# Justin-Huber/SfM-project

Measured on AMD Instinct MI355X. Metric: verified matches/sec (match+RANSAC), higher is better.
Workload: dtype int8 MFMA -> exact int32 (K1), f32 (K2); 1 GPU; cfg4: all 124750 unordered pairs of 500 synthetic images x 4096 128-D u8 SIFT-like descriptors; L2 match (mutual cross check + ratio 4/5) + 8-point RANSAC 4096 hyp/pair (seed 42, Sampson 1 px^2, min 15 inliers); launches of <= 131072 pairs; n_img=500, k=4096, n_hyp=4096, pairs_total=124750, pairs_rank0=124750, launches_rank0=1, parallelism=pair-sharded dp1

## Files before the change

include/sfmcore.h:

```cpp
#ifndef SFMCORE_H
#define SFMCORE_H

#include <stdint.h>

#ifdef __cplusplus
extern "C" {
#endif

#define SFM_OK 0
#define SFM_ERR_INVALID (-1)
#define SFM_ERR_HIP (-2)
#define SFM_ERR_NOMEM (-3)

#define SFM_METRIC_L2 0
#define SFM_METRIC_HAMMING 1

#define SFM_XC_NONE 0
#define SFM_XC_MUTUAL 1
#define SFM_XC_OPENCV 2

typedef struct sfm_ctx sfm_ctx;

typedef struct sfm_match_params {
    int32_t metric;
// ... 118 lines not shown
               int32_t* out_n_tracks, int32_t* out_track_ptr, int32_t* out_track_img,
               int32_t* out_track_kp);

int sfm_triangulate(sfm_ctx* ctx, int32_t n_cam, const double* cams, const double* pp,
                    int32_t n_pt, const int32_t* pt_ptr, const int32_t* cam_idx, const double* uv,
                    double* out_pts, double* out_stats);

typedef struct sfm_register_params {
    int32_t n_hyp;
    int32_t refine;
    double thr;
    uint64_t seed;
} sfm_register_params;

int sfm_register_batch(sfm_ctx* ctx, int32_t n_img, const int32_t* corr_ptr, const double* xy,
                       const double* X, const double* intr, const int32_t* img_id,
                       const sfm_register_params* prm, double* out_cams, int32_t* out_count,
                       int32_t* out_key, uint8_t* out_mask);

typedef struct sfm_orb_params {
    int32_t n_features;
    int32_t n_levels;
    double scale_factor;
    int32_t fast_threshold;
    int32_t _pad;
} sfm_orb_params;

int sfm_orb_batch(sfm_ctx* ctx, const uint8_t* images, int32_t n_img, int32_t H, int32_t W,
                  const sfm_orb_params* prm, float* out_kp, uint8_t* out_desc,
                  int32_t* out_count);

int sfm_calib_mfma_i8(sfm_ctx* ctx, float target_ms, double* out);

#ifdef __cplusplus
}
#endif
#endif
```

sfm-project_amd/csrc/capi.hip:

```cpp
#include "sfm_internal.h"

static thread_local std::string g_err;

namespace sfm {
void set_error(const std::string& msg) { g_err = msg; }

void* workspace(sfm_ctx* ctx, size_t bytes) {
    ctx->rs_last_w = nullptr;
    ctx->rs_last_pairs = ctx->rs_last_hyp = 0;
    if (bytes <= ctx->ws_bytes) return ctx->ws;
    hipStreamCaptureStatus cap = hipStreamCaptureStatusNone;
    if (hipStreamIsCapturing(ctx->stream, &cap) == hipSuccess && cap != hipStreamCaptureStatusNone) {
        set_error("workspace growth to " + std::to_string(bytes) +
                  " bytes while the context's stream is being captured: run the call once "
                  "uncaptured first so the workspace is sized");
        return nullptr;
    }
    if (ctx->ws) {
        (void)hipStreamSynchronize(ctx->stream);
        (void)hipFree(ctx->ws);
        ctx->ws = nullptr;
        ctx->ws_bytes = 0;
    }
    size_t want = align_up(bytes + bytes / 4, 1 << 20);
// ... 24 lines not shown
    if (std::string(prop.gcnArchName).rfind("gfx950", 0) != 0) {
        sfm::set_error(std::string("sfm_ctx_create: libsfmcore is built for gfx950, device is ") +
                       prop.gcnArchName);
        return SFM_ERR_INVALID;
    }
    sfm_ctx* c = new sfm_ctx();
    c->device = device;
    c->n_cu = prop.multiProcessorCount;
    if (hipStreamCreateWithFlags(&c->own_stream, hipStreamNonBlocking) != hipSuccess) {
        delete c;
        sfm::set_error("sfm_ctx_create: hipStreamCreate failed");
        return SFM_ERR_HIP;
    }
    if (hipEventCreateWithFlags(&c->handoff, hipEventDisableTiming) != hipSuccess) {
        (void)hipStreamDestroy(c->own_stream);
        delete c;
        sfm::set_error("sfm_ctx_create: hipEventCreate failed");
        return SFM_ERR_HIP;
    }
    c->stream = c->own_stream;
    *out = c;
    return SFM_OK;
}

int sfm_ctx_destroy(sfm_ctx* ctx) {
    if (!ctx) return SFM_OK;
    (void)hipSetDevice(ctx->device);
    if (ctx->stream) (void)hipStreamSynchronize(ctx->stream);
    if (ctx->ws) (void)hipFree(ctx->ws);
    if (ctx->handoff) (void)hipEventDestroy(ctx->handoff);
    if (ctx->pinned) (void)hipHostFree(ctx->pinned);
    if (ctx->poll_ev) (void)hipEventDestroy(ctx->poll_ev);
    if (ctx->rs_acc) (void)hipFree(ctx->rs_acc);
    if (ctx->own_stream) (void)hipStreamDestroy(ctx->own_stream);
    delete ctx;
    return SFM_OK;
}

int sfm_ctx_set_stream(sfm_ctx* ctx, void* hip_stream) {
    SFM_REQUIRE(ctx != nullptr, "sfm_ctx_set_stream: ctx is NULL");
    hipStream_t s = (hipStream_t)hip_stream;
    if (s == ctx->stream) return SFM_OK;
    SFM_HIP_CHECK(hipSetDevice(ctx->device));
    SFM_HIP_CHECK(hipEventRecord(ctx->handoff, ctx->stream));
    SFM_HIP_CHECK(hipStreamWaitEvent(s, ctx->handoff, 0));
    ctx->stream = s;
    return SFM_OK;
}

int sfm_ctx_sync(sfm_ctx* ctx) {
    SFM_REQUIRE(ctx != nullptr, "sfm_ctx_sync: ctx is NULL");
    SFM_HIP_CHECK(hipSetDevice(ctx->device));
    SFM_HIP_CHECK(hipStreamSynchronize(ctx->stream));
    return SFM_OK;
}

int sfm_match_batch(sfm_ctx* ctx, const uint8_t* desc, const int32_t* n_kp, int32_t n_img,
                    int32_t k_max, int32_t dim, const int32_t* pairs, int32_t n_pairs,
                    const sfm_match_params* prm, int32_t* out_count, int32_t* out_match,
                    int32_t* out_dist) {
    SFM_REQUIRE(ctx && prm, "sfm_match_batch: ctx/prm is NULL");
    SFM_REQUIRE(n_pairs >= 0 && n_img >= 0 && k_max >= 0, "sfm_match_batch: negative size");
    if (n_pairs == 0) return SFM_OK;
    SFM_REQUIRE(desc && n_kp && pairs && out_count && out_match && out_dist,
                "sfm_match_batch: NULL array");
    SFM_REQUIRE(prm->cross_check >= 0 && prm->cross_check <= 2, "sfm_match_batch: bad cross_check");
// ... 54 lines not shown
```

sfm-project_amd/csrc/match_l2fr.hip:

```cpp
#include <algorithm>
#include <climits>
#include <cstdlib>

#include "match_common.h"

namespace {

typedef int v4i __attribute__((ext_vector_type(4)));
typedef int v16i __attribute__((ext_vector_type(16)));
typedef __attribute__((address_space(3))) void lds_void;
typedef const __attribute__((address_space(1))) void gbl_void;

constexpr int D = 128;
#ifndef L2FR_WAVES
#define L2FR_WAVES 8
#endif
constexpr int WAVES = L2FR_WAVES;
constexpr int SCAN_THREADS = 64 * WAVES;
#ifndef L2FR_QT
#define L2FR_QT 4
#endif
constexpr int QT = L2FR_QT;
constexpr int QB = WAVES * QT * 32;
constexpr int SCAN_MIN_WAVES = 8 / QT;
// ... 677 lines not shown
            crec[tid] = fw[q];
            cA[tid] = norm[(size_t)a * k_pad + q];
        }
        __syncthreads();
        for (int c = g; c < nbat; c += 8) {
            const int q = cq[c];
            const int4 r = crec[c];
            const int row = (r.z - tg) * 32 + t, j = r.z * 32 + t;
            const uint4* x = &qrows[c * SLOTS];
            const uint4* y = &tiles[row * SLOTS];
            int dot = 0;
#pragma unroll
            for (int k = 0; k < SLOTS; ++k) {
                const uint4 u = x[k], v = y[k ^ (row & 7)];
                dot = __builtin_amdgcn_sdot4((int)u.x, (int)v.x, dot, false);
                dot = __builtin_amdgcn_sdot4((int)u.y, (int)v.y, dot, false);
                dot = __builtin_amdgcn_sdot4((int)u.z, (int)v.z, dot, false);
                dot = __builtin_amdgcn_sdot4((int)u.w, (int)v.w, dot, false);
            }
            const bool hit = (j < nb) && (dot + tci[row] == r.x);
            const unsigned long long bal = __ballot(hit);
            const unsigned m = (unsigned)(bal >> (32 * (g & 1)));
            if (t == 0 && m == 0) qs[q] = make_int4(ST_SLOW, 0, 0, 0);
            if (m != 0 && t == __builtin_ctz(m)) {
                const long long A = cA[c];
                const long long d1 = A - (2LL * dot - tnb[row]);
                const long long d2lo = r.y > E_VALID ? A - 2LL * r.y - 1 : sfm::DIST_INF;
                const long long d2hi = r.y > E_VALID ? A - 2LL * r.y : sfm::DIST_INF;
                int st;
                if (max_dist >= 0 && !(d1 < max_dist)) st = ST_DROP;
                else if (sfm::ratio_ok(d1, d2lo, rnum, rden, true)) st = ST_PASS;
                else if (!sfm::ratio_ok(d1, d2hi, rnum, rden, true)) st = ST_DROP;
                else st = ST_SLOW;
                qs[q] = make_int4(st, j, (int)d1, 0);
            }
        }
        __syncthreads();
    }
}

#ifndef L2FR_REC_SB
#define L2FR_REC_SB 2
#endif
constexpr int REC_SB = L2FR_REC_SB;
__global__ __launch_bounds__(256, REC_SB > 2 ? 2 : 3) void l2fr_recover_mfma_kernel(
    const uint8_t* __restrict__ desc, int k_max, int k_pad, const int32_t* __restrict__ norm,
    const int32_t* __restrict__ cinit, const int4* __restrict__ rinfo,
    const int32_t* __restrict__ n_rng, const int4* __restrict__ fwd,
    const uint8_t* __restrict__ cls, int rnum, int rden, long long max_dist,
    int4* __restrict__ qst) {
    __shared__ unsigned short clist[REC_R * KMAX];
    __shared__ __attribute__((aligned(16))) int gini[GROUP];
    __shared__ unsigned char gpar[GROUP];
    __shared__ unsigned long long wlo[4], whi[4];
    __shared__ int toff[9];
    const int ri = blockIdx.x, grp = blockIdx.y, tid = threadIdx.x;
    if (ri >= *n_rng) return;
    const int wave = tid >> 6, lane = tid & 63, h = lane >> 5, r32 = lane & 31;
    int4 pi[REC_R];
#pragma unroll
    for (int e = 0; e < REC_R; ++e) pi[e] = rinfo[(size_t)ri * REC_R + e];
    const int b = pi[0].z, nb = pi[0].w >> 16;
    const int ntiles = (nb + 31) >> 5, tg = grp * 8;
    if (nb <= 0 || tg >= ntiles) return;
    const uint8_t* db = desc + (size_t)b * k_max * D;

    uint4 cv[REC_R];
// ... 126 lines not shown
#pragma unroll
            for (int u = 0; u < 2; ++u) {
                v16i acc;
                const int* gi = gini + (2 * wave + u) * 32 + 4 * h;
#pragma unroll
                for (int g = 0; g < 4; ++g) {
                    const v4i c4 = *(const v4i*)(gi + 8 * g);
                    acc[4 * g + 0] = c4.x; acc[4 * g + 1] = c4.y;
                    acc[4 * g + 2] = c4.z; acc[4 * g + 3] = c4.w;
                }
#pragma unroll
                for (int s = 0; s < NK; ++s)
                    acc = __builtin_amdgcn_mfma_i32_32x32x32_i8(af[u][s], bf[k][s], acc, 0, 0, 0);
#pragma unroll
                for (int rr = 0; rr < 16; ++rr)
                    hit = (mine == u && acc[rr] == r.x) ? 8 * (rr >> 2) + 4 * h + (rr & 3) : hit;
            }
            hit = max(hit, __shfl_xor(hit, 32));
            if (h == 0 && qq[k] >= 0) {
                int4* qs = qst + (size_t)pp[k] * k_pad;
                if (hit < 0) {
                    qs[qq[k]] = make_int4(ST_SLOW, 0, 0, 0);
                } else {
                    const int jg = (2 * wave + mine) * 32 + hit;
                    const long long A = AA[k];
                    const long long d1 = A - 2LL * r.x - gpar[jg];
                    const long long d2lo = r.y > E_VALID ? A - 2LL * r.y - 1 : sfm::DIST_INF;
                    const long long d2hi = r.y > E_VALID ? A - 2LL * r.y : sfm::DIST_INF;
                    int st;
                    if (max_dist >= 0 && !(d1 < max_dist)) st = ST_DROP;
                    else if (sfm::ratio_ok(d1, d2lo, rnum, rden, true)) st = ST_PASS;
                    else if (!sfm::ratio_ok(d1, d2hi, rnum, rden, true)) st = ST_DROP;
                    else st = ST_SLOW;
                    qs[qq[k]] = make_int4(st, tg * 32 + jg, (int)d1, 0);
                }
            }
        }
    }
}

__global__ __launch_bounds__(256) void l2fr_compact_kernel(
    const uint8_t* __restrict__ desc, const int32_t* __restrict__ n_kp, int k_max, int k_pad,
    const int32_t* __restrict__ norm, const int32_t* __restrict__ pairs,
    const int4* __restrict__ qst, int rnum, int rden, long long max_dist,
    int4* __restrict__ surv, int32_t* __restrict__ scount, int32_t* __restrict__ out_count,
    int32_t* __restrict__ out_match, int32_t* __restrict__ out_dist) {
    __shared__ Top2 red[256];
    __shared__ int slow[256];
    __shared__ int nslow, wsum[8];
    const int p = blockIdx.x, tid = threadIdx.x;
    const int a = pairs[2 * p], b = pairs[2 * p + 1];
    const int na = n_kp[a], nb = n_kp[b];
    const bool direct = out_count != nullptr;
    int32_t* om = direct ? out_match + (size_t)p * k_max * 2 : nullptr;
    int32_t* od = direct ? out_dist + (size_t)p * k_max : nullptr;
    if (na <= 0 || nb <= 0) {
        if (tid == 0) {
            if (direct) out_count[p] = 0;
            else scount[p] = 0;
        }
        return;
    }
    const int4* qs = qst + (size_t)p * k_pad;
    const int32_t* na_norm = norm + (size_t)a * k_pad;
    const int32_t* nb_norm = norm + (size_t)b * k_pad;
    const uint4* qa = (const uint4*)(desc + (size_t)a * k_max * D);
    const uint8_t* db = desc + (size_t)b * k_max * D;
    int4* sv = surv + (size_t)p * k_pad;
    int base = 0;
    for (int q0 = 0; q0 < na; q0 += 256) {
        const int q = q0 + tid;
        int4 r = (q < na) ? qs[q] : make_int4(ST_DROP, 0, 0, 0);
        if (tid == 0) nslow = 0;
        __syncthreads();
        if (r.x == ST_SLOW) slow[atomicAdd(&nslow, 1)] = tid;
        __syncthreads();
        const int ns = nslow;
        for (int i = 0; i < ns; ++i) {
            const int who = slow[i], qq = q0 + who;
            const Top2 e = exact_row_scan(qa + (size_t)qq * SLOTS, db, nb_norm, nb, na_norm[qq], red);
            if (tid == who) {
                bool keep = sfm::ratio_ok(e.b1, e.b2, rnum, rden, true);
                keep = keep && (max_dist < 0 || e.b1 < max_dist);
                r = make_int4(keep ? ST_PASS : ST_DROP, e.j1, (int)e.b1, 0);
            }
        }
        const bool keep = r.x == ST_PASS;
        if (direct)
            base = sfm::compact256(keep, q, r.y, r.z, base, wsum, om, od);
        else
            base = compact_rec(keep, make_int4(q, r.y, r.z, 0), base, wsum, sv);
    }
    if (tid == 0) {
        if (direct) out_count[p] = base;
        else scount[p] = base;
    }
}

__global__ __launch_bounds__(256) void l2fr_final_kernel(
    const uint8_t* __restrict__ desc, const int32_t* __restrict__ n_kp, int k_max, int k_pad,
    const int32_t* __restrict__ norm, const int32_t* __restrict__ cinit,
    const int32_t* __restrict__ pairs, const int4* __restrict__ surv,
    const int32_t* __restrict__ scount, const int4* __restrict__ rev, int mutual,
    int32_t* __restrict__ out_count, int32_t* __restrict__ out_match,
    int32_t* __restrict__ out_dist) {
    __shared__ int wsum[8];
    __shared__ int amb[256];
    __shared__ int namb;
    __shared__ unsigned char keepx[256];
    __shared__ long long redd[256];
    __shared__ int redq[256];
    const int p = blockIdx.x, tid = threadIdx.x;
    const int a = pairs[2 * p], b = pairs[2 * p + 1];
    const int na = n_kp[a], nb = n_kp[b];
    const int S = (na > 0 && nb > 0) ? scount[p] : 0;
    const int4* sv = surv + (size_t)p * k_pad;
    const int4* rv = rev + (size_t)p * k_pad;
    const int32_t* na_norm = norm + (size_t)a * k_pad;
    const int32_t* nb_norm = norm + (size_t)b * k_pad;
    const int32_t* ca = cinit + (size_t)a * k_pad;
    const uint8_t* da = desc + (size_t)a * k_max * D;
    const uint4* dbv = (const uint4*)(desc + (size_t)b * k_max * D);
    int32_t* om = out_match + (size_t)p * k_max * 2;
    int32_t* od = out_dist + (size_t)p * k_max;
    int base = 0;
    for (int k0 = 0; k0 < S; k0 += 256) {
        const int k = k0 + tid;
        int4 s = make_int4(0, 0, 0, 0);
        bool keep = false;
        if (tid == 0) namb = 0;
        __syncthreads();
        if (k < S) {
            s = sv[k];
            keep = true;
            if (mutual) {
                const int4 r = rv[k];
                const int dot = (int)(((long long)na_norm[s.x] + nb_norm[s.y] - s.z) >> 1);
                const int ep = dot + ca[s.x];
                keep = (ep == r.x) && (r.y < r.x);
                if (ep == r.x && r.y == r.x) amb[atomicAdd(&namb, 1)] = tid;
            }
        }
        keepx[tid] = keep;
        __syncthreads();
        const int nam = namb;
// ... 41 lines not shown
        const int4 r = rec[(size_t)p * k_pad + i];
        out_match[((size_t)p * k_max + i) * 2] = r.x;
        out_match[((size_t)p * k_max + i) * 2 + 1] = r.y;
        out_dist[(size_t)p * k_max + i] = r.z;
    }
    if (threadIdx.x == 0) out_count[p] = n;
}

}

int sfm_match_l2fr_launch(sfm_ctx* ctx, const uint8_t* desc, const int32_t* n_kp, int32_t n_img,
                          int32_t k_max, const int32_t* pairs, int32_t n_pairs,
                          const sfm_match_params* prm, int32_t* out_count, int32_t* out_match,
                          int32_t* out_dist) {
    hipStream_t st = ctx->stream;
    if (k_max == 0) {
        SFM_HIP_CHECK(hipMemsetAsync(out_count, 0, sizeof(int32_t) * n_pairs, st));
        return SFM_OK;
    }
    const int k_pad = (int)sfm::align_up((size_t)k_max, KALIGN);
    SFM_REQUIRE(k_pad <= KMAX, "sfm_match_batch: L2 matcher needs k_max <= 4096");
    const int n_qblk = (k_max + QB - 1) / QB;
    const size_t tab = (size_t)n_img * k_pad * sizeof(int32_t);
    const size_t recb = (size_t)n_pairs * k_pad * sizeof(int4);
    const size_t cntb = sfm::align_up(sizeof(int32_t) * (size_t)n_pairs, 256);
    const size_t descb = sfm::align_up((size_t)n_img * k_max * D, 256);
    const size_t ordb = sfm::align_up(sizeof(int32_t) * (size_t)n_pairs, 256);
    const size_t clsb = sfm::align_up((size_t)n_pairs * k_pad, 256);
    const int n_rng_max = n_pairs / REC_R + n_img + 1;
    const size_t rngb = sfm::align_up(sizeof(int2) * (size_t)n_rng_max, 256);
    const size_t rinfob = sizeof(int4) * (size_t)n_rng_max * REC_R;
    const size_t sinfob = sfm::align_up(sizeof(int4) * (size_t)n_pairs, 256);
    const size_t uinfob = sfm::align_up(UNIT * sizeof(int4) * (size_t)n_pairs, 256);
    char* ws = (char*)sfm::workspace(ctx, 256 + 2 * tab + 3 * recb + cntb + descb + 2 * ordb + clsb +
                                              256 + rngb + rinfob + 256 + sinfob + uinfob + 256);
    if (!ws) return SFM_ERR_NOMEM;
    char* w = ws;
    uint8_t* zero_row = (uint8_t*)w; w += 256;
    int32_t* norm = (int32_t*)w; w += tab;
    int32_t* cinit = (int32_t*)w; w += tab;
    int4* fwd = (int4*)w; w += recb;
    int4* surv = (int4*)w; w += recb;
    int4* rev = (int4*)w; w += recb;
    int32_t* scount = (int32_t*)w; w += cntb;
    uint8_t* desc_i8 = (uint8_t*)w; w += descb;
    int32_t* ord_f = (int32_t*)w; w += ordb;
    int32_t* ord_r = (int32_t*)w; w += ordb;
    uint8_t* cls = (uint8_t*)w; w += clsb;
    int32_t* n_rng = (int32_t*)w; w += 256;
    int2* rng = (int2*)w; w += rngb;
    int4* rinfo = (int4*)w; w += rinfob;
    int4* sinfo_f = (int4*)sfm::align_up((size_t)w, 256);
    int4* uinfo = (int4*)((char*)sinfo_f + sinfob);
    int32_t* n_units = (int32_t*)((char*)uinfo + uinfob);
    static const bool units_env = [] {
        const char* e = getenv("SFM_L2FR_UNITS");
        return !(e && e[0] == '0');
    }();
    const bool units = units_env && (3 * (size_t)n_img + 2) * sizeof(int) <= 65536;
    const int ppx = (n_pairs + 7) / 8;
    const int n_blk = n_pairs;
    const int grid = 8 * ppx * n_qblk;
    const bool mutual = prm->cross_check == SFM_XC_MUTUAL;

    const int32_t* sord_f = ord_f;
    const int32_t* sord_r = ord_r;
    const int unit_blk = units ? (mutual ? 2 : 1) : -1;
    const int bpi = (k_pad + 1023) / 1024, n_prep = bpi * n_img;
    hipLaunchKernelGGL(l2fr_setup_kernel, dim3(n_prep + (mutual ? 2 : 1) + (units ? 1 : 0)),
                       dim3(1024), ((units ? 3 : 2) * (size_t)n_img + 2) * sizeof(int), st, n_prep,
                       bpi, desc, n_kp, k_max, k_pad, norm, cinit, zero_row, (uint4*)desc_i8, pairs,
                       n_pairs, n_img, ord_f, ord_r, rng, n_rng, rinfo, sinfo_f, unit_blk, uinfo,
                       n_units);
    SFM_HIP_CHECK(hipGetLastError());
    int4* qst = rev;
    const FwdCls fc{norm, prm->ratio_num, prm->ratio_den, (long long)prm->max_dist, qst, cls};
    hipLaunchKernelGGL(l2fr_scan_kernel<false>, dim3(grid), dim3(SCAN_THREADS), 0, st, desc_i8, n_kp, k_max,
                       k_pad, cinit, zero_row, pairs, n_qblk, sord_f,
                       (const int4*)(units ? uinfo : sinfo_f), n_blk, (const int4*)nullptr,
                       (const int32_t*)nullptr, fwd, fc, (const int32_t*)(units ? n_units : nullptr));
    SFM_HIP_CHECK(hipGetLastError());
    const char* dbg = getenv("SFM_L2FR_DEBUG");
    const int dmode = dbg ? atoi(dbg) : 0;
    if (dmode == 1) {
        hipLaunchKernelGGL(l2fr_dump_kernel, dim3(n_pairs), dim3(256), 0, st, n_kp, pairs, k_max,
                           k_pad, (const int4*)fwd, (const int32_t*)nullptr, out_count, out_match,
                           out_dist);
        return SFM_OK;
    }
#ifdef L2FR_RECOVER_VALU
    hipLaunchKernelGGL(l2fr_recover_kernel, dim3(n_pairs, k_pad / GROUP), dim3(256), 0, st, desc_i8,
                       n_kp, k_max, k_pad, norm, cinit, pairs, fwd, (const uint8_t*)cls,
                       prm->ratio_num, prm->ratio_den, (long long)prm->max_dist, qst);
#else
    hipLaunchKernelGGL(l2fr_recover_mfma_kernel, dim3(n_rng_max, k_pad / GROUP), dim3(256), 0, st,
                       desc_i8, k_max, k_pad, norm, cinit, (const int4*)rinfo, (const int32_t*)n_rng,
                       (const int4*)fwd, (const uint8_t*)cls, prm->ratio_num, prm->ratio_den,
                       (long long)prm->max_dist, qst);
#endif
    SFM_HIP_CHECK(hipGetLastError());
    const bool direct = !mutual && dmode == 0;
    hipLaunchKernelGGL(l2fr_compact_kernel, dim3(n_pairs), dim3(256), 0, st, desc_i8, n_kp, k_max,
                       k_pad, norm, pairs, (const int4*)qst, prm->ratio_num, prm->ratio_den,
                       (long long)prm->max_dist, surv, scount, direct ? out_count : nullptr,
                       out_match, out_dist);
    SFM_HIP_CHECK(hipGetLastError());
    if (direct) return SFM_OK;
    if (dmode == 2) {
        hipLaunchKernelGGL(l2fr_dump_kernel, dim3(n_pairs), dim3(256), 0, st, n_kp, pairs, k_max,
                           k_pad, (const int4*)surv, (const int32_t*)scount, out_count, out_match,
                           out_dist);
        return SFM_OK;
    }
    if (mutual) {
        hipLaunchKernelGGL(l2fr_scan_kernel<true>, dim3(grid), dim3(SCAN_THREADS), 0, st, desc_i8, n_kp,
                           k_max, k_pad, cinit, zero_row, pairs, n_qblk, sord_r,
                           (const int4*)nullptr, n_blk,
                           (const int4*)surv, (const int32_t*)scount, rev, fc,
                           (const int32_t*)nullptr);
        SFM_HIP_CHECK(hipGetLastError());
    }
    if (dmode == 3) {
        hipLaunchKernelGGL(l2fr_dump_kernel, dim3(n_pairs), dim3(256), 0, st, n_kp, pairs, k_max,
                           k_pad, (const int4*)rev, (const int32_t*)scount, out_count, out_match,
                           out_dist);
        return SFM_OK;
    }
    hipLaunchKernelGGL(l2fr_final_kernel, dim3(n_pairs), dim3(256), 0, st, desc_i8, n_kp, k_max,
                       k_pad, norm, cinit, pairs, surv, scount, rev, mutual ? 1 : 0, out_count,
                       out_match, out_dist);
    SFM_HIP_CHECK(hipGetLastError());
    return SFM_OK;
}

#ifdef L2FR_CLOCK
extern "C" int sfm_debug_l2fr_stamps(unsigned long long* host, int32_t n_blocks) {
    const size_t n = L2FR_CLOCK_W * (size_t)std::min(n_blocks, L2FR_CLOCK_SLOTS);
    SFM_HIP_CHECK(hipDeviceSynchronize());
    SFM_HIP_CHECK(hipMemcpyFromSymbol(host, HIP_SYMBOL(g_l2fr_clock), n * sizeof(unsigned long long)));
    return SFM_OK;
}
#endif
```

sfm-project_amd/csrc/match_mfma.hip:

```cpp
#include <algorithm>
#include <climits>
#include <cstdlib>
#include <cstring>

#include "match_common.h"

namespace {

typedef int v4i __attribute__((ext_vector_type(4)));
typedef int v16i __attribute__((ext_vector_type(16)));

constexpr int WAVES = 8;
constexpr int STAGE_BYTES = 32768;
constexpr int KALIGN = 256;
constexpr int KMAX_L2 = 4096;
constexpr int KMAX_MU = 8192;

template <int D> struct Geo {
    static constexpr int QT = D == 128 ? 4 : 2;
    static constexpr int QB = WAVES * QT * 32;
    static constexpr int CHUNK = STAGE_BYTES / D;
    static constexpr int NK = D / 32;
    static constexpr int SLOTS = D / 16;
};
// ... 1272 lines not shown
        hipLaunchKernelGGL((mfma_match_kernel<256, false>), dim3(grid), dim3(512), 0, st, desc_i8,
                           n_kp, k_max, k_pad, norm, crow, zero_row, pairs, n_qblk, pair_order,
                           n_blk, rowres, colpart);
    }
    SFM_HIP_CHECK(hipGetLastError());
    hipLaunchKernelGGL(both_finalize_kernel, dim3(n_pairs), dim3(256), (size_t)k_pad * 8, st, n_kp,
                       k_max, k_pad, norm, pairs, n_pairs, n_qblk, rowres, colpart,
                       prm->cross_check, (long long)prm->max_dist, out_count, out_match, out_dist,
                       2);
    SFM_HIP_CHECK(hipGetLastError());
    return SFM_OK;
}

int sfm_match_both_launch(sfm_ctx* ctx, int metric, const uint8_t* desc, const int32_t* n_kp,
                          int32_t n_img, int32_t k_max, const int32_t* pairs, int32_t n_pairs,
                          const sfm_match_params* prm, int32_t* out_count, int32_t* out_match,
                          int32_t* out_dist) {
    return match_tile_launch(ctx, metric, desc, n_kp, n_img, k_max, pairs, n_pairs, prm, out_count,
                             out_match, out_dist, 2);
}

int sfm_match_l2_launch(sfm_ctx* ctx, const uint8_t* desc, const int32_t* n_kp, int32_t n_img,
                        int32_t k_max, const int32_t* pairs, int32_t n_pairs,
                        const sfm_match_params* prm, int32_t* out_count, int32_t* out_match,
                        int32_t* out_dist) {
    const char* pe = getenv("SFM_L2_PATH");
    const bool ratio = prm->ratio_den > 0;
    if (pe && strcmp(pe, "fused") == 0)
        return mfma_match_launch(ctx, SFM_METRIC_L2, desc, n_kp, n_img, k_max, pairs, n_pairs, prm,
                                 out_count, out_match, out_dist);
    if (pe && strcmp(pe, "fr") == 0 && ratio && prm->cross_check != SFM_XC_OPENCV)
        return sfm_match_l2fr_launch(ctx, desc, n_kp, n_img, k_max, pairs, n_pairs, prm,
                                     out_count, out_match, out_dist);
    if (prm->cross_check != SFM_XC_NONE)
        return mfma_mutual_launch(ctx, SFM_METRIC_L2, desc, n_kp, n_img, k_max, pairs, n_pairs,
                                  prm, out_count, out_match, out_dist);
    if (ratio)
        return sfm_match_l2fr_launch(ctx, desc, n_kp, n_img, k_max, pairs, n_pairs, prm,
                                     out_count, out_match, out_dist);
    return mfma_match_launch(ctx, SFM_METRIC_L2, desc, n_kp, n_img, k_max, pairs, n_pairs, prm,
                             out_count, out_match, out_dist);
}

int sfm_match_hamming_mfma_launch(sfm_ctx* ctx, const uint8_t* desc, const int32_t* n_kp,
                                  int32_t n_img, int32_t k_max, const int32_t* pairs,
                                  int32_t n_pairs, const sfm_match_params* prm,
                                  int32_t* out_count, int32_t* out_match, int32_t* out_dist) {
    const char* pe = getenv("SFM_HAMMING_PATH");
    if (prm->ratio_den == 0 && !(pe && (strcmp(pe, "mutual") == 0 || strcmp(pe, "fused") == 0)))
        return match_tile_launch(ctx, SFM_METRIC_HAMMING, desc, n_kp, n_img, k_max, pairs, n_pairs,
                                 prm, out_count, out_match, out_dist, 1);
    const bool col = pe && strcmp(pe, "mutual") == 0 ? prm->cross_check != SFM_XC_NONE
                                                    : prm->cross_check == SFM_XC_OPENCV;
    if (col && !(pe && strcmp(pe, "fused") == 0))
        return mfma_mutual_launch(ctx, SFM_METRIC_HAMMING, desc, n_kp, n_img, k_max, pairs,
                                  n_pairs, prm, out_count, out_match, out_dist);
    return mfma_match_launch(ctx, SFM_METRIC_HAMMING, desc, n_kp, n_img, k_max, pairs, n_pairs,
                             prm, out_count, out_match, out_dist);
}

#ifdef MU_CLOCK
extern "C" int sfm_debug_clock_stamps(unsigned long long* host, int32_t n_blocks) {
    const size_t n = MU_CLOCK_W * (size_t)std::min(n_blocks, MU_CLOCK_SLOTS);
    SFM_HIP_CHECK(hipDeviceSynchronize());
    SFM_HIP_CHECK(hipMemcpyFromSymbol(host, HIP_SYMBOL(g_mu_clock), n * sizeof(unsigned long long)));
    return SFM_OK;
// ... 3 lines not shown
```

sfm-project_amd/csrc/sfm_internal.h:

```cpp
#pragma once
#include <hip/hip_runtime.h>
#include <stdint.h>
#include <string>

#include "../../include/sfmcore.h"

struct sfm_ctx {
    int device = 0;
    hipStream_t own_stream = nullptr;
    hipStream_t stream = nullptr;
    void* ws = nullptr;
    size_t ws_bytes = 0;
    hipEvent_t handoff = nullptr;
    int32_t* pinned = nullptr;
    hipEvent_t poll_ev = nullptr;
    int n_cu = 256;
    int ransac_stats = 0;
    unsigned long long* rs_acc = nullptr;
    const uint32_t* rs_last_w = nullptr;
    int rs_last_pairs = 0, rs_last_hyp = 0;
    int ba_nchunk = 0, ba_ntotal = 0;
    int32_t ba_chunk_pt[17] = {0}, ba_chunk_obs[17] = {0};
    const int32_t* ba_cam_bounds = nullptr;
    int ba_nslot = 0, ba_nseg = 0, ba_ninst = 0, ba_nent = 0, ba_ngroup = 0;
    const int32_t *ba_slot_cam = nullptr, *ba_seg = nullptr, *ba_inst = nullptr,
                  *ba_row_ptr = nullptr, *ba_row_ent = nullptr, *ba_sg_ptr = nullptr,
                  *ba_sg = nullptr, *ba_gk = nullptr;
};

namespace sfm {

struct ChunkOff {
    int32_t v[17];
};
__device__ __forceinline__ int chunk_of(int x, int nck, const ChunkOff& off, const ChunkOff& base,
                                        int& a, int& b) {
    int k = 0;
    a = base.v[0];
    b = base.v[1];
#pragma unroll
    for (int i = 1; i < 16; ++i) {
        if (i < nck && x >= off.v[i]) {
            k = i;
            a = base.v[i];
            b = base.v[i + 1];
        }
    }
    return k;
}
__device__ __forceinline__ double chunk_tree16(double (&a)[16]) {
#pragma unroll
    for (int w = 8; w >= 1; w >>= 1)
#pragma unroll
// ... 85 lines not shown
```

sfm-project_amd/sfmcore.py:

```python
from __future__ import annotations

import ctypes as C
import os
import threading

import numpy as np

_HERE = os.path.dirname(os.path.abspath(__file__))
LIB_PATH = os.environ.get("SFMCORE_LIB") or os.path.join(_HERE, "lib", "libsfmcore.so")

METRIC_L2, METRIC_HAMMING = 0, 1
XC_NONE, XC_MUTUAL, XC_OPENCV = 0, 1, 2

EXPORTED = ["sfm_ctx_create", "sfm_ctx_destroy", "sfm_ctx_set_stream", "sfm_ctx_sync",
            "sfm_last_error", "sfm_version", "sfm_match_batch", "sfm_ransac_f_batch",
            "sfm_ba_jtj", "sfm_graph_offsets", "sfm_graph_rows", "sfm_ba_solve", "sfm_ba_cost",
            "sfm_ba_update", "sfm_tracks", "sfm_triangulate", "sfm_register_batch",
            "sfm_ba_fix_params", "sfm_orb_batch", "sfm_ransac_counts", "sfm_ba_solve_stage",
            "sfm_ransac_stats", "sfm_ransac_f_batch_f64", "sfm_graph_rows_packed",
            "sfm_graph_expand", "sfm_match_batch_both", "sfm_ransac_wave_stops",
            "sfm_ba_set_chunks", "sfm_ba_chunk_tree", "sfm_ba_set_schur", "sfm_calib_mfma_i8"]


class SfmCoreError(RuntimeError):
    pass


class MatchParams(C.Structure):
    _fields_ = [("metric", C.c_int32), ("cross_check", C.c_int32), ("ratio_num", C.c_int32),
                ("ratio_den", C.c_int32), ("max_dist", C.c_int64)]


class BaSolveParams(C.Structure):
    _fields_ = [("lam", C.c_double), ("tol", C.c_double), ("max_iter", C.c_int32),
                ("poll", C.c_int32), ("poll_first", C.c_int32)]


class RegisterParams(C.Structure):
    _fields_ = [("n_hyp", C.c_int32), ("refine", C.c_int32), ("thr", C.c_double),
                ("seed", C.c_uint64)]


class OrbParams(C.Structure):
    _fields_ = [("n_features", C.c_int32), ("n_levels", C.c_int32), ("scale_factor", C.c_double),
                ("fast_threshold", C.c_int32), ("_pad", C.c_int32)]


class RansacParams(C.Structure):
    _fields_ = [("n_hyp", C.c_int32), ("min_inliers", C.c_int32), ("thr", C.c_float),
                ("_pad", C.c_int32), ("seed", C.c_uint64)]


(BA_STAGE_SETUP, BA_STAGE_SETUP_FINISH, BA_STAGE_ITER, BA_STAGE_ITER_FINISH, BA_STAGE_BACKSUB,
 BA_STAGE_MODEL, BA_STAGE_POLL, BA_STAGE_SCHUR) = range(8)
# ... 3 lines not shown
_lock = threading.Lock()


def load_library(path: str = LIB_PATH):
    global _lib
    with _lock:
        if _lib is not None:
            return _lib
        import torch
        if not os.path.exists(path):
            if os.path.exists("/opt/rocm/bin/hipcc"):
                from build_lib import build
                build()
            if not os.path.exists(path):
                raise SfmCoreError(f"libsfmcore.so not found at {path}; run __graft_entry__.build()")
        L = C.CDLL(path)
        vp, i32, i64, f64 = C.c_void_p, C.c_int32, C.c_int64, C.c_double
        L.sfm_ctx_create.argtypes = [i32, C.POINTER(vp)]
        L.sfm_ctx_destroy.argtypes = [vp]
        L.sfm_ctx_set_stream.argtypes = [vp, vp]
        L.sfm_ctx_sync.argtypes = [vp]
        L.sfm_last_error.restype = C.c_char_p
        L.sfm_version.restype = i32
        L.sfm_match_batch.argtypes = [vp, vp, vp, i32, i32, i32, vp, i32, C.POINTER(MatchParams),
                                      vp, vp, vp]
        L.sfm_match_batch_both.argtypes = L.sfm_match_batch.argtypes
        L.sfm_ransac_f_batch.argtypes = [vp, vp, i32, i32, vp, i32, vp, vp,
                                         C.POINTER(RansacParams), vp, vp, vp, vp, vp]
        L.sfm_ransac_f_batch_f64.argtypes = L.sfm_ransac_f_batch.argtypes
        L.sfm_ransac_counts.argtypes = [vp, vp, i32, i32, vp, i32, vp, vp,
                                        C.POINTER(RansacParams), vp, vp, vp, vp]
        L.sfm_ransac_stats.argtypes = [vp, i32, vp]
        L.sfm_ransac_wave_stops.argtypes = [vp, i32, i32, vp]
        L.sfm_calib_mfma_i8.argtypes = [vp, C.c_float, vp]
        L.sfm_ba_jtj.argtypes = [vp, i32, vp, vp, i32, vp, i32, vp, vp, vp, vp, vp, vp, f64, vp,
                                 vp, vp, vp, vp, vp, vp]
        L.sfm_ba_solve.argtypes = [vp, i32, i32, i32, vp, vp, vp, vp, vp, vp, vp, vp, vp, vp,
                                   C.POINTER(BaSolveParams), vp, vp, vp]
        L.sfm_ba_solve_stage.argtypes = [vp, i32, i32, i32, i32, i32, vp, vp, vp, vp, vp, vp, vp,
                                         vp, vp, vp, C.POINTER(BaSolveParams), vp, vp, vp, vp, vp]
        L.sfm_ba_cost.argtypes = [vp, i32, vp, vp, i32, vp, i32, vp, vp, vp, f64, vp]
        L.sfm_ba_update.argtypes = [vp, i32, vp, vp, i32, vp, vp, vp, vp]
        L.sfm_ba_fix_params.argtypes = [vp, i32, i32, vp, vp, vp, vp, vp]
        L.sfm_ba_set_chunks.argtypes = [vp, i32, vp, vp, i32, vp]
        L.sfm_ba_set_schur.argtypes = [vp, i32, vp, i32, vp, i32, vp, vp, i32, vp, i32, vp, vp, vp]
        L.sfm_ba_chunk_tree.argtypes = [vp, i32, i64, vp, vp]
        L.sfm_orb_batch.argtypes = [vp, vp, i32, i32, i32, C.POINTER(OrbParams), vp, vp, vp]
        L.sfm_register_batch.argtypes = [vp, i32, vp, vp, vp, vp, vp, C.POINTER(RegisterParams),
                                         vp, vp, vp, vp]
        L.sfm_triangulate.argtypes = [vp, i32, vp, vp, i32, vp, vp, vp, vp, vp]
        L.sfm_tracks.argtypes = [vp, i32, vp, i32, vp, i64, vp, i32, vp, vp, vp, vp]
        L.sfm_graph_offsets.argtypes = [vp, i32, vp, i32, vp]
        L.sfm_graph_rows.argtypes = [vp, i32, i32, i32, vp, vp, vp, vp, i32, vp, vp]
        L.sfm_graph_rows_packed.argtypes = [vp, i32, i32, vp, vp, vp, vp, i32, vp, vp]
        L.sfm_graph_expand.argtypes = [vp, i32, i32, vp, vp, vp, vp, vp]
        for name in EXPORTED:
            getattr(L, name).restype = getattr(L, name).restype or C.c_int
        _lib = L
        return L


def _check(rc: int):
    if rc != 0:
        msg = load_library().sfm_last_error().decode(errors="replace")
        raise SfmCoreError(f"libsfmcore error {rc}: {msg}")

# ... 124 lines not shown
        prm = RansacParams(int(n_hyp), int(min_inliers), float(thr), 0, int(seed))
        self._bind_stream()
        fn = self.lib.sfm_ransac_f_batch_f64 if f64 else self.lib.sfm_ransac_f_batch
        _check(fn(self.handle, _ptr(kps), n_img, k_max, _ptr(pairs), P,
                                           _ptr(count), _ptr(match), C.byref(prm),
                                           _ptr(out["inl_count"]), _ptr(out["best_h"]),
                                           _ptr(out["mask"]), _ptr(out["F"]), _ptr(out["norm"])))
        return out

    def ransac_counts(self, kps, pairs, count, match, n_hyp=4096, seed=42, thr=1.0,
                      hyp_F=False, hyp_mask=False):
        torch = self.torch
        n_img, k_max, _ = kps.shape
        P = pairs.shape[0]
        dev = kps.device
        if kps.dtype != torch.float32 or not kps.is_contiguous():
            raise SfmCoreError("ransac_counts: kps must be contiguous float32")
        counts = torch.empty((P, n_hyp), dtype=torch.int32, device=dev)
        norm = torch.empty((P, 6), dtype=torch.float32, device=dev)
        F = torch.empty((P, n_hyp, 9), dtype=torch.float32, device=dev) if hyp_F else None
        mk = torch.zeros((P, n_hyp, k_max), dtype=torch.uint8, device=dev) if hyp_mask else None
        prm = RansacParams(int(n_hyp), 0, float(thr), 0, int(seed))
        self._bind_stream()
        _check(self.lib.sfm_ransac_counts(self.handle, _ptr(kps), n_img, k_max, _ptr(pairs), P,
                                          _ptr(count), _ptr(match), C.byref(prm), _ptr(counts),
                                          _ptr(norm), _ptr(F) if hyp_F else None,
                                          _ptr(mk) if hyp_mask else None))
        return (counts, norm, F, mk) if (hyp_F or hyp_mask) else (counts, norm)

    def ransac_stats(self, enable=True, read=False):
        out = (C.c_uint64 * 3)()
        self._bind_stream()
        _check(self.lib.sfm_ransac_stats(self.handle, 1 if enable else 0, out if read else None))
        return (int(out[0]), int(out[1]), int(out[2])) if read else None

    def ransac_wave_stops(self, n_pairs, n_hyp):
        out = np.zeros((n_pairs, n_hyp // 64), np.uint32)
        self._bind_stream()
        _check(self.lib.sfm_ransac_wave_stops(self.handle, int(n_pairs), int(n_hyp),
                                              out.ctypes.data_as(C.c_void_p)))
        return out

    def calib_mfma_i8(self, target_ms=200.0):
        out = np.zeros(4, np.float64)
        self._bind_stream()
        _check(self.lib.sfm_calib_mfma_i8(self.handle, float(target_ms),
                                          out.ctypes.data_as(C.c_void_p)))
        return {"ms": float(out[0]), "tops": float(out[1]), "clock_ghz": float(out[2]),
                "frac_nominal": float(out[3])}

    def graph_rows(self, pair_base, count, match, inl_count, mask, min_inliers=15,
                   return_offsets=False, packed=False):
        torch = self.torch
        P, k_max = mask.shape
        dev = mask.device
        offs = torch.empty(P + 1, dtype=torch.int64, device=dev)
        self._bind_stream()
        _check(self.lib.sfm_graph_offsets(self.handle, P, _ptr(inl_count), int(min_inliers),
                                          _ptr(offs)))
        n = int(offs[P].item())
        rows = torch.empty((n,) if packed else (n, 3), dtype=torch.int32, device=dev)
        if n and packed:
            _check(self.lib.sfm_graph_rows_packed(self.handle, P, k_max, _ptr(count),
                                                  _ptr(match), _ptr(mask), _ptr(inl_count),
                                                  int(min_inliers), _ptr(offs), _ptr(rows)))
        elif n:
# ... 307 lines not shown
```

Before: 228.0 million verified matches/s.

## Route mutual L2 matching through l2fr path with per-pair mutual certification kernel

Sends mutual-cross-check ratio matching with k_max between 1536 and 4096 through the forward-ratio (l2fr) pipeline by default, instead of the MFMA mutual path. Adds a certification kernel that uses distance lower bounds to find the few query rows that could beat each surviving match, checks only those with exact dot products, and finalises the pair directly. Pairs it certifies get a zero reverse count, so the reverse scan has little to do for them, and the final kernel skips them via a flag. Pairs whose threat count exceeds the cap fall back to the full reverse scan, so the change adds one extra kernel launch and some workspace in exchange for skipping most of the reverse-direction work.

```diff
diff --git a/include/sfmcore.h b/include/sfmcore.h
--- a/include/sfmcore.h
+++ b/include/sfmcore.h
@@ -174,6 +174,8 @@
 
 int sfm_calib_mfma_i8(sfm_ctx* ctx, float target_ms, double* out);
 
+int sfm_match_cert_stats(sfm_ctx* ctx, int32_t enable, uint64_t* out);
+
 #ifdef __cplusplus
 }
 #endif
diff --git a/sfm-project_amd/csrc/capi.hip b/sfm-project_amd/csrc/capi.hip
--- a/sfm-project_amd/csrc/capi.hip
+++ b/sfm-project_amd/csrc/capi.hip
@@ -80,6 +80,7 @@
     if (ctx->pinned) (void)hipHostFree(ctx->pinned);
     if (ctx->poll_ev) (void)hipEventDestroy(ctx->poll_ev);
     if (ctx->rs_acc) (void)hipFree(ctx->rs_acc);
+    if (ctx->cert_acc) (void)hipFree(ctx->cert_acc);
     if (ctx->own_stream) (void)hipStreamDestroy(ctx->own_stream);
     delete ctx;
     return SFM_OK;
diff --git a/sfm-project_amd/csrc/match_l2fr.hip b/sfm-project_amd/csrc/match_l2fr.hip
--- a/sfm-project_amd/csrc/match_l2fr.hip
+++ b/sfm-project_amd/csrc/match_l2fr.hip
@@ -733,7 +733,7 @@
                 else if (sfm::ratio_ok(d1, d2lo, rnum, rden, true)) st = ST_PASS;
                 else if (!sfm::ratio_ok(d1, d2hi, rnum, rden, true)) st = ST_DROP;
                 else st = ST_SLOW;
-                qs[q] = make_int4(st, j, (int)d1, 0);
+                qs[q] = make_int4(st, j, (int)d1, 1);
             }
         }
         __syncthreads();
@@ -926,7 +926,7 @@
                     else if (sfm::ratio_ok(d1, d2lo, rnum, rden, true)) st = ST_PASS;
                     else if (!sfm::ratio_ok(d1, d2hi, rnum, rden, true)) st = ST_DROP;
                     else st = ST_SLOW;
-                    qs[qq[k]] = make_int4(st, tg * 32 + jg, (int)d1, 0);
+                    qs[qq[k]] = make_int4(st, tg * 32 + jg, (int)d1, 1);
                 }
             }
         }
@@ -936,7 +936,7 @@
 __global__ __launch_bounds__(256) void l2fr_compact_kernel(
     const uint8_t* __restrict__ desc, const int32_t* __restrict__ n_kp, int k_max, int k_pad,
     const int32_t* __restrict__ norm, const int32_t* __restrict__ pairs,
-    const int4* __restrict__ qst, int rnum, int rden, long long max_dist,
+    int4* __restrict__ qst, int rnum, int rden, long long max_dist,
     int4* __restrict__ surv, int32_t* __restrict__ scount, int32_t* __restrict__ out_count,
     int32_t* __restrict__ out_match, int32_t* __restrict__ out_dist) {
     __shared__ Top2 red[256];
@@ -955,7 +955,7 @@
         }
         return;
     }
-    const int4* qs = qst + (size_t)p * k_pad;
+    int4* qs = qst + (size_t)p * k_pad;
     const int32_t* na_norm = norm + (size_t)a * k_pad;
     const int32_t* nb_norm = norm + (size_t)b * k_pad;
     const uint4* qa = (const uint4*)(desc + (size_t)a * k_max * D);
@@ -976,7 +976,8 @@
             if (tid == who) {
                 bool keep = sfm::ratio_ok(e.b1, e.b2, rnum, rden, true);
                 keep = keep && (max_dist < 0 || e.b1 < max_dist);
-                r = make_int4(keep ? ST_PASS : ST_DROP, e.j1, (int)e.b1, 0);
+                r = make_int4(keep ? ST_PASS : ST_DROP, e.j1, (int)e.b1, 1);
+                if (!direct) qs[qq] = r;
             }
         }
         const bool keep = r.x == ST_PASS;
@@ -991,13 +992,137 @@
     }
 }
 
+constexpr int CERT_TMAX = 2048;
+constexpr long long CERT_CAP_DEFAULT = 16384;
+
+__global__ __launch_bounds__(256) void l2fr_mutual_cert_kernel(
+    const uint8_t* __restrict__ desc, const int32_t* __restrict__ n_kp, int k_max, int k_pad,
+    const int32_t* __restrict__ norm, const int32_t* __restrict__ pairs,
+    const int4* __restrict__ fwd, const int4* __restrict__ qst, const int4* __restrict__ surv,
+    const int32_t* __restrict__ scount, long long cap, int32_t* __restrict__ rcount,
+    uint8_t* __restrict__ flag, unsigned long long* __restrict__ stats,
+    int32_t* __restrict__ out_count, int32_t* __restrict__ out_match,
+    int32_t* __restrict__ out_dist) {
+    __shared__ unsigned long long owner[KMAX];
+    __shared__ int tbound[CERT_TMAX];
+    __shared__ unsigned short tq[CERT_TMAX];
+    __shared__ unsigned char killed[KMAX];
+    __shared__ int wmax[4], wsum[8];
+    __shared__ int nthreat;
+    const int p = blockIdx.x, tid = threadIdx.x;
+    const int a = pairs[2 * p], b = pairs[2 * p + 1];
+    const int na = n_kp[a], nb = n_kp[b];
+    const int S = (na > 0 && nb > 0) ? scount[p] : 0;
+    if (cap <= 0) {
+        if (tid == 0) {
+            rcount[p] = S;
+            flag[p] = 1;
+            if (stats) atomicAdd(&stats[1], 1ull);
+        }
+        return;
+    }
+    if (S == 0) {
+        if (tid == 0) {
+            rcount[p] = 0;
+            flag[p] = 0;
+            out_count[p] = 0;
+            if (stats) atomicAdd(&stats[0], 1ull);
+        }
+        return;
+    }
+    const int4* fw = fwd + (size_t)p * k_pad;
+    const int4* qs = qst + (size_t)p * k_pad;
+    const int4* sv = surv + (size_t)p * k_pad;
+    const int32_t* na_norm = norm + (size_t)a * k_pad;
+    const int32_t* nb_norm = norm + (size_t)b * k_pad;
+    const uint4* qa = (const uint4*)(desc + (size_t)a * k_max * D);
+    const uint4* dbv = (const uint4*)(desc + (size_t)b * k_max * D);
+
+    int tmax = 0;
+    for (int k = tid; k < S; k += 256) {
+        tmax = max(tmax, sv[k].z);
+        killed[k] = 0;
+    }
+    for (int j = tid; j < nb; j += 256) owner[j] = ~0ull;
+#pragma unroll
+    for (int m = 32; m > 0; m >>= 1) tmax = max(tmax, __shfl_xor(tmax, m));
+    if ((tid & 63) == 0) wmax[tid >> 6] = tmax;
+    if (tid == 0) nthreat = 0;
+    __syncthreads();
+    const long long T = max(max(wmax[0], wmax[1]), max(wmax[2], wmax[3]));
+
+    for (int q = tid; q < na; q += 256) {
+        const int4 r = qs[q];
+        const int4 f = fw[q];
+        const long long A = na_norm[q];
+        long long bound;
+        if (r.w == 1) {
+            if ((unsigned)r.y < (unsigned)nb)
+                atomicMin(&owner[r.y], ((unsigned long long)(unsigned)r.z << 32) | (unsigned)q);
+            bound = f.y > E_VALID ? A - 2LL * f.y - 1 : sfm::DIST_INF;
+        } else {
+            bound = A - 2LL * f.x - 1;
+        }
+        if (bound <= T) {
+            const int i = atomicAdd(&nthreat, 1);
+            if (i < CERT_TMAX) {
+                tq[i] = (unsigned short)q;
+                tbound[i] = (int)bound;
+            }
+        }
+    }
+    __syncthreads();
+    const int nT = nthreat;
+    if (nT > CERT_TMAX || (long long)nT * S > cap) {
+        if (tid == 0) {
+            rcount[p] = S;
+            flag[p] = 1;
+            if (stats) atomicAdd(&stats[1], 1ull);
+        }
+        return;
+    }
+    unsigned dots = 0;
+    for (int i = tid; i < nT * S; i += 256) {
+        const int t = i / S, k = i - t * S;
+        const int4 s = sv[k];
+        const int qp = tq[t];
+        if (qp == s.x || s.z < tbound[t]) continue;
+        const int dot = dot128(qa + (size_t)qp * SLOTS, dbv + (size_t)s.y * SLOTS);
+        const long long d = (long long)na_norm[qp] + nb_norm[s.y] - 2LL * dot;
+        if (d < s.z || (d == s.z && qp < s.x)) killed[k] = 1;
+        ++dots;
+    }
+    if (stats && dots) atomicAdd(&stats[2], (unsigned long long)dots);
+    __syncthreads();
+    int32_t* om = out_match + (size_t)p * k_max * 2;
+    int32_t* od = out_dist + (size_t)p * k_max;
+    int base = 0;
+    for (int k0 = 0; k0 < S; k0 += 256) {
+        const int k = k0 + tid;
+        int4 s = make_int4(0, 0, 0, 0);
+        bool keep = false;
+        if (k < S) {
+            s = sv[k];
+            keep = !killed[k] &&
+                   owner[s.y] == (((unsigned long long)(unsigned)s.z << 32) | (unsigned)s.x);
+        }
+        base = sfm::compact256(keep, s.x, s.y, s.z, base, wsum, om, od);
+    }
+    if (tid == 0) {
+        out_count[p] = base;
+        rcount[p] = 0;
+        flag[p] = 0;
+        if (stats) atomicAdd(&stats[0], 1ull);
+    }
+}
+
 __global__ __launch_bounds__(256) void l2fr_final_kernel(
     const uint8_t* __restrict__ desc, const int32_t* __restrict__ n_kp, int k_max, int k_pad,
     const int32_t* __restrict__ norm, const int32_t* __restrict__ cinit,
     const int32_t* __restrict__ pairs, const int4* __restrict__ surv,
     const int32_t* __restrict__ scount, const int4* __restrict__ rev, int mutual,
-    int32_t* __restrict__ out_count, int32_t* __restrict__ out_match,
-    int32_t* __restrict__ out_dist) {
+    const uint8_t* __restrict__ flag, int32_t* __restrict__ out_count,
+    int32_t* __restrict__ out_match, int32_t* __restrict__ out_dist) {
     __shared__ int wsum[8];
     __shared__ int amb[256];
     __shared__ int namb;
@@ -1005,6 +1130,7 @@
     __shared__ long long redd[256];
     __shared__ int redq[256];
     const int p = blockIdx.x, tid = threadIdx.x;
+    if (flag && !flag[p]) return;
     const int a = pairs[2 * p], b = pairs[2 * p + 1];
     const int na = n_kp[a], nb = n_kp[b];
     const int S = (na > 0 && nb > 0) ? scount[p] : 0;
@@ -1112,8 +1238,10 @@
     const size_t rinfob = sizeof(int4) * (size_t)n_rng_max * REC_R;
     const size_t sinfob = sfm::align_up(sizeof(int4) * (size_t)n_pairs, 256);
     const size_t uinfob = sfm::align_up(UNIT * sizeof(int4) * (size_t)n_pairs, 256);
+    const size_t flagb = sfm::align_up((size_t)n_pairs, 256);
     char* ws = (char*)sfm::workspace(ctx, 256 + 2 * tab + 3 * recb + cntb + descb + 2 * ordb + clsb +
-                                              256 + rngb + rinfob + 256 + sinfob + uinfob + 256);
+                                              256 + rngb + rinfob + 256 + sinfob + uinfob + 256 +
+                                              cntb + flagb);
     if (!ws) return SFM_ERR_NOMEM;
     char* w = ws;
     uint8_t* zero_row = (uint8_t*)w; w += 256;
@@ -1133,6 +1261,8 @@
     int4* sinfo_f = (int4*)sfm::align_up((size_t)w, 256);
     int4* uinfo = (int4*)((char*)sinfo_f + sinfob);
     int32_t* n_units = (int32_t*)((char*)uinfo + uinfob);
+    int32_t* rcount = (int32_t*)((char*)n_units + 256);
+    uint8_t* flag = (uint8_t*)rcount + cntb;
     static const bool units_env = [] {
         const char* e = getenv("SFM_L2FR_UNITS");
         return !(e && e[0] == '0');
@@ -1181,7 +1311,7 @@
     SFM_HIP_CHECK(hipGetLastError());
     const bool direct = !mutual && dmode == 0;
     hipLaunchKernelGGL(l2fr_compact_kernel, dim3(n_pairs), dim3(256), 0, st, desc_i8, n_kp, k_max,
-                       k_pad, norm, pairs, (const int4*)qst, prm->ratio_num, prm->ratio_den,
+                       k_pad, norm, pairs, qst, prm->ratio_num, prm->ratio_den,
                        (long long)prm->max_dist, surv, scount, direct ? out_count : nullptr,
                        out_match, out_dist);
     SFM_HIP_CHECK(hipGetLastError());
@@ -1192,11 +1322,25 @@
                            out_dist);
         return SFM_OK;
     }
+    const char* ce = getenv("SFM_L2FR_CERT");
+    const bool cert = mutual && dmode == 0 && !(ce && ce[0] == '0');
+    if (cert) {
+        const char* cc = getenv("SFM_L2FR_CERT_CAP");
+        const long long cap = cc ? atoll(cc) : CERT_CAP_DEFAULT;
+        unsigned long long* stats = ctx->cert_stats ? ctx->cert_acc : nullptr;
+        if (stats)
+            SFM_HIP_CHECK(hipMemsetAsync(stats, 0, 3 * sizeof(unsigned long long), st));
+        hipLaunchKernelGGL(l2fr_mutual_cert_kernel, dim3(n_pairs), dim3(256), 0, st, desc_i8, n_kp,
+                           k_max, k_pad, norm, pairs, (const int4*)fwd, (const int4*)qst,
+                           (const int4*)surv, (const int32_t*)scount, cap, rcount, flag, stats,
+                           out_count, out_match, out_dist);
+        SFM_HIP_CHECK(hipGetLastError());
+    }
     if (mutual) {
         hipLaunchKernelGGL(l2fr_scan_kernel<true>, dim3(grid), dim3(SCAN_THREADS), 0, st, desc_i8, n_kp,
                            k_max, k_pad, cinit, zero_row, pairs, n_qblk, sord_r,
                            (const int4*)nullptr, n_blk,
-                           (const int4*)surv, (const int32_t*)scount, rev, fc,
+                           (const int4*)surv, (const int32_t*)(cert ? rcount : scount), rev, fc,
                            (const int32_t*)nullptr);
         SFM_HIP_CHECK(hipGetLastError());
     }
@@ -1207,9 +1351,26 @@
         return SFM_OK;
     }
     hipLaunchKernelGGL(l2fr_final_kernel, dim3(n_pairs), dim3(256), 0, st, desc_i8, n_kp, k_max,
-                       k_pad, norm, cinit, pairs, surv, scount, rev, mutual ? 1 : 0, out_count,
-                       out_match, out_dist);
+                       k_pad, norm, cinit, pairs, surv, scount, rev, mutual ? 1 : 0,
+                       (const uint8_t*)(cert ? flag : nullptr), out_count, out_match, out_dist);
     SFM_HIP_CHECK(hipGetLastError());
+    return SFM_OK;
+}
+
+extern "C" int sfm_match_cert_stats(sfm_ctx* ctx, int32_t enable, uint64_t* out) {
+    SFM_REQUIRE(ctx, "sfm_match_cert_stats: ctx is NULL");
+    SFM_HIP_CHECK(hipSetDevice(ctx->device));
+    if (!ctx->cert_acc) {
+        SFM_HIP_CHECK(hipMalloc(&ctx->cert_acc, 3 * sizeof(unsigned long long)));
+        SFM_HIP_CHECK(hipMemsetAsync(ctx->cert_acc, 0, 3 * sizeof(unsigned long long), ctx->stream));
+    }
+    if (out) {
+        unsigned long long h[3];
+        SFM_HIP_CHECK(hipMemcpyAsync(h, ctx->cert_acc, sizeof(h), hipMemcpyDeviceToHost, ctx->stream));
+        SFM_HIP_CHECK(hipStreamSynchronize(ctx->stream));
+        out[0] = h[0]; out[1] = h[1]; out[2] = h[2];
+    }
+    ctx->cert_stats = enable ? 1 : 0;
     return SFM_OK;
 }
 
diff --git a/sfm-project_amd/csrc/match_mfma.hip b/sfm-project_amd/csrc/match_mfma.hip
--- a/sfm-project_amd/csrc/match_mfma.hip
+++ b/sfm-project_amd/csrc/match_mfma.hip
@@ -1328,6 +1328,10 @@
     if (pe && strcmp(pe, "fr") == 0 && ratio && prm->cross_check != SFM_XC_OPENCV)
         return sfm_match_l2fr_launch(ctx, desc, n_kp, n_img, k_max, pairs, n_pairs, prm,
                                      out_count, out_match, out_dist);
+    if (prm->cross_check == SFM_XC_MUTUAL && ratio && k_max > 1536 && k_max <= 4096 &&
+        !(pe && strcmp(pe, "mutual") == 0))
+        return sfm_match_l2fr_launch(ctx, desc, n_kp, n_img, k_max, pairs, n_pairs, prm,
+                                     out_count, out_match, out_dist);
     if (prm->cross_check != SFM_XC_NONE)
         return mfma_mutual_launch(ctx, SFM_METRIC_L2, desc, n_kp, n_img, k_max, pairs, n_pairs,
                                   prm, out_count, out_match, out_dist);
diff --git a/sfm-project_amd/csrc/sfm_internal.h b/sfm-project_amd/csrc/sfm_internal.h
--- a/sfm-project_amd/csrc/sfm_internal.h
+++ b/sfm-project_amd/csrc/sfm_internal.h
@@ -19,6 +19,8 @@
     unsigned long long* rs_acc = nullptr;
     const uint32_t* rs_last_w = nullptr;
     int rs_last_pairs = 0, rs_last_hyp = 0;
+    int cert_stats = 0;
+    unsigned long long* cert_acc = nullptr;
     int ba_nchunk = 0, ba_ntotal = 0;
     int32_t ba_chunk_pt[17] = {0}, ba_chunk_obs[17] = {0};
     const int32_t* ba_cam_bounds = nullptr;
diff --git a/sfm-project_amd/sfmcore.py b/sfm-project_amd/sfmcore.py
--- a/sfm-project_amd/sfmcore.py
+++ b/sfm-project_amd/sfmcore.py
@@ -19,7 +19,8 @@
             "sfm_ba_fix_params", "sfm_orb_batch", "sfm_ransac_counts", "sfm_ba_solve_stage",
             "sfm_ransac_stats", "sfm_ransac_f_batch_f64", "sfm_graph_rows_packed",
             "sfm_graph_expand", "sfm_match_batch_both", "sfm_ransac_wave_stops",
-            "sfm_ba_set_chunks", "sfm_ba_chunk_tree", "sfm_ba_set_schur", "sfm_calib_mfma_i8"]
+            "sfm_ba_set_chunks", "sfm_ba_chunk_tree", "sfm_ba_set_schur", "sfm_calib_mfma_i8",
+            "sfm_match_cert_stats"]
 
 
 class SfmCoreError(RuntimeError):
@@ -89,6 +90,7 @@
                                         C.POINTER(RansacParams), vp, vp, vp, vp]
         L.sfm_ransac_stats.argtypes = [vp, i32, vp]
         L.sfm_ransac_wave_stops.argtypes = [vp, i32, i32, vp]
+        L.sfm_match_cert_stats.argtypes = [vp, i32, vp]
         L.sfm_calib_mfma_i8.argtypes = [vp, C.c_float, vp]
         L.sfm_ba_jtj.argtypes = [vp, i32, vp, vp, i32, vp, i32, vp, vp, vp, vp, vp, vp, f64, vp,
                                  vp, vp, vp, vp, vp, vp]
@@ -279,6 +281,13 @@
         out = (C.c_uint64 * 3)()
         self._bind_stream()
         _check(self.lib.sfm_ransac_stats(self.handle, 1 if enable else 0, out if read else None))
+        return (int(out[0]), int(out[1]), int(out[2])) if read else None
+
+    def match_cert_stats(self, enable=True, read=False):
+        out = (C.c_uint64 * 3)()
+        self._bind_stream()
+        _check(self.lib.sfm_match_cert_stats(self.handle, 1 if enable else 0,
+                                             out if read else None))
         return (int(out[0]), int(out[1]), int(out[2])) if read else None
 
     def ransac_wave_stops(self, n_pairs, n_hyp):
```

Result: faster. 264.7 million verified matches/s, median of 6 (+16.1%).
